# wdykas/LDDL

Measured on AMD Instinct MI355X. Metric: WordPiece+MLM tokens/sec (1/2/4/8 MI355X) and % of HBM roofline, higher is better.
Workload: dtype uint16

## Files before the change

lddl_amd/csrc/tokenize.hip:

```cpp
#include <algorithm>
#include <cstdlib>
#include <cstring>
#include <type_traits>
#include <vector>
#include <cstdio>

#include "common.h"
#include "ctx.h"
#include "device.h"
#include "lddl_amd.h"

namespace lddl {
namespace {

constexpr int kBlock = 128;
constexpr int kWordStride = 420;

__device__ inline uint32_t tab_entry(const Tables& T, uint32_t cp) {
  if (cp > 0x10FFFF) return kDrop << 30;
  return T.pages[(uint32_t)T.l1[cp >> 8] * 256u + (cp & 255u)];
}

__device__ inline uint32_t utf8_next(const uint8_t* b, int64_t end, int64_t& i) {
  const uint32_t c = b[i];
// ... 165 lines not shown
__device__ inline uint64_t lanes_below() { return (1ull << lane_id()) - 1ull; }

__device__ inline int match_special_at(const Tables& T, const uint8_t* b, int64_t i, int64_t end) {
  for (int k = 0; k < kNumSpecial; ++k)
    if (T.special_id[k] >= 0 && match_special(b, i, end, k)) return k;
  return -1;
}

struct B32 {
  uint64_t w0, w1, w2, w3;
};

__device__ inline B32 shr_bytes(const B32& v, int s) {
  const int q = s >> 3, r = (s & 7) * 8;
  uint64_t a0 = q == 0 ? v.w0 : q == 1 ? v.w1 : q == 2 ? v.w2 : v.w3;
  uint64_t a1 = q == 0 ? v.w1 : q == 1 ? v.w2 : q == 2 ? v.w3 : 0ull;
  uint64_t a2 = q == 0 ? v.w2 : q == 1 ? v.w3 : 0ull;
  uint64_t a3 = q == 0 ? v.w3 : 0ull;
  if (r) {
    a0 = (a0 >> r) | (a1 << (64 - r));
    a1 = (a1 >> r) | (a2 << (64 - r));
    a2 = (a2 >> r) | (a3 << (64 - r));
    a3 >>= r;
  }
  return B32{a0, a1, a2, a3};
}

struct Pcs {
  int32_t* b;
  __device__ void put(int n, int32_t v) { b[64 * n] = v; }
  __device__ int32_t get(int q) const { return b[64 * q]; }
};

struct TokStats {
#ifdef LDDL_STAMPS
  uint64_t c[10];
  __device__ void add(int i, uint64_t v) { c[i] += v; }
  __device__ void wave(int i) {
    const uint64_t m = __builtin_amdgcn_ballot_w64(true);
    if ((uint32_t)__lane_id() == (uint32_t)__builtin_ctzll(m)) c[i] += 1;
  }
#else
  __device__ void add(int, uint64_t) {}
  __device__ void wave(int) {}
#endif
};

__device__ inline bool tail_match(const Tables& T, int32_t id, const B32& a, int len) {
  const ulonglong2* p = reinterpret_cast<const ulonglong2*>(T.vlong + 4 * (int64_t)id);
  const ulonglong2 lo = p[0], hi = p[1];
  const uint64_t d = keep_bytes(lo.y ^ a.w1, len - 8) | keep_bytes(hi.x ^ a.w2, len - 16) |
                     keep_bytes(hi.y ^ a.w3, len - 24);
  return d == 0;
}


struct Probe {
  uint64_t k0;
  uint32_t k1, want, slot;
  VEnt e;
};
__device__ inline Probe probe_first(const Tables& T, const B32& a, int len, uint32_t cont) {
  Probe q;
  q.k0 = keep_bytes(a.w0, len);
  q.k1 = (uint32_t)keep_bytes(a.w1, len - 8 < 4 ? len - 8 : 4);
  q.want = kMetaValid | (cont ? kMetaCont : 0u) | (len > 12 ? kMetaLong : 0u) | ((uint32_t)len << 21);
  q.slot = (uint32_t)vhash(q.k0, q.k1, len, cont) & T.vmask;
  q.e = T.vhash[q.slot];
  return q;
// ... 254 lines not shown
  while (j < je) {
    const uint32_t b0 = text[j];
    uint32_t cp, e;
    if (b0 < 0x80) {
      cp = b0;
      e = s_ascii[b0];
      ++j;
    } else {
      cp = utf8_next(text, je, j);
      e = tab_entry(T, cp);
    }
    if ((e >> 30) == kDrop) continue;
    uint8_t ob[12];
    int olen;
    if (e & kIdent) olen = put_utf8(ob, cp);
    else if (e & kMulti) {
      const uint8_t* p = T.pool + (e & 0xFFFFFFu);
      olen = p[0];
      for (int q = 0; q < olen; ++q) ob[q] = p[2 + q];
    } else olen = put_utf8(ob, e & 0x1FFFFFu);
    if (nb + olen > kNorm) return -1;
    for (int q = 0; q < olen; ++q) w[nb + q] = ob[q];
    nb += olen;
  }
  if (nb == 0) return 0;
  uint64_t ends = 1ull << nb;
  for (int e = 1; e < nb; ++e)
    if ((w[e] & 0xC0) != 0x80) ends |= 1ull << e;
  const uint64_t* w8 = reinterpret_cast<const uint64_t*>(w);
  const B32 v{w8[0], w8[1], w8[2], w8[3]};
  return wordpiece32(T, bloom, v, nb, ends, pc);
}

struct UnitWord {
  B32 v;
  int nb;
  uint64_t ends;
  int status;
};

__device__ UnitWord unit_word(const Tables& T, const uint32_t* s_ascii, const uint8_t* __restrict__ text,
                              int64_t n_bytes, int64_t start, int len, bool unit_slow, uint8_t* w) {
  UnitWord u;
  u.status = 0;
  if (!unit_slow && len <= 32 && T.ascii_mode != 0) {
    B32 v = load32(text, n_bytes, start);
    if (T.ascii_mode == 1) v = B32{swar_lower(v.w0), swar_lower(v.w1), swar_lower(v.w2), swar_lower(v.w3)};
    u.v = v;
    u.nb = len;
    u.ends = ~0ull;
    return u;
  }
  int nb = 0;
  int64_t j = start;
  const int64_t je = start + len;
  while (j < je) {
    const uint32_t b0 = text[j];
    uint32_t cp, e;
    if (b0 < 0x80) {
      cp = b0;
      e = s_ascii[b0];
      ++j;
    } else {
      cp = utf8_next(text, je, j);
      e = tab_entry(T, cp);
    }
    if ((e >> 30) == kDrop) continue;
    uint8_t ob[12];
    int olen;
    if (e & kIdent) olen = put_utf8(ob, cp);
    else if (e & kMulti) {
      const uint8_t* p = T.pool + (e & 0xFFFFFFu);
      olen = p[0];
      for (int q = 0; q < olen; ++q) ob[q] = p[2 + q];
    } else olen = put_utf8(ob, e & 0x1FFFFFu);
    if (nb + olen > kNorm) {
      u.status = -1;
      return u;
    }
    for (int q = 0; q < olen; ++q) w[nb + q] = ob[q];
    nb += olen;
  }
  u.nb = nb;
  if (nb == 0) {
    u.status = 1;
    return u;
  }
  uint64_t ends = 1ull << nb;
  for (int e = 1; e < nb; ++e)
    if ((w[e] & 0xC0) != 0x80) ends |= 1ull << e;
  u.ends = ends;
  const uint64_t* w8 = reinterpret_cast<const uint64_t*>(w);
  u.v = B32{w8[0], w8[1], w8[2], w8[3]};
  return u;
}

__global__ void __launch_bounds__(64 * kTW) tokenize_wave_kernel(
    Tables T, const uint8_t* __restrict__ text, int64_t n_bytes, const int64_t* __restrict__ sent_off,
    int64_t n_sent, int32_t max_pieces, int32_t* __restrict__ ids, int32_t* __restrict__ sent_len,
    int32_t* __restrict__ fb_list, uint32_t* __restrict__ fb_n) {
  __shared__ uint32_t s_ascii[128];
  __shared__ WaveLds s_w[kTW];
  for (int c = threadIdx.x; c < 128; c += blockDim.x) s_ascii[c] = tab_entry(T, (uint32_t)c);
  __syncthreads();
  const int lane = lane_id();
  WaveLds& W = s_w[threadIdx.x >> 6];
  const int64_t stride = (int64_t)gridDim.x * kTW;
  for (int64_t s = (int64_t)blockIdx.x * kTW + wave_id(); s < n_sent; s += stride) {
    const int64_t b0 = sent_off[s], b1 = sent_off[s + 1];
    int64_t pos = b0;
    int32_t emitted = 0, flags = 0;
    bool fallback = false;
    while (pos < b1 && emitted < max_pieces) {
      const uint32_t byte = pos + lane < b1 ? text[pos + lane] : 0x20u;
      const WinResult R = classify_window(T, s_ascii, text, pos, b1, byte);
      if (R.fallback) { fallback = true; break; }
      store_units(R, W);
      int npc = 0;
      bool cs_flag = false;
      Pcs pc{W.pcs + lane};
      if (lane < R.n_units) {
        const int us = W.us[lane], ue = W.ue[lane], kind = W.uk[lane];
        const int ulen = ue - us + 1;
        const bool unit_slow = ((R.slow >> us) & (ulen >= 64 ? ~0ull : ((1ull << ulen) - 1))) != 0;
        npc = unit_pieces(T, T.bloom, s_ascii, text, n_bytes, pos + us, ulen, kind, unit_slow, pc,
                          W.nrm + lane * kNorm, cs_flag);
// ... 13 lines not shown
    } else if (lane == 0) {
      sent_len[s] = (emitted < max_pieces ? emitted : max_pieces) | flags;
    }
  }
}

enum : int { kMemoOff = 0, kMemoBuild = 1, kMemoLookup = 2 };
constexpr int kMemoLog2 = 22;
constexpr int kMemoDiv = 32;
struct WordMemo {
  uint4* tab;
  uint32_t mask;
};
constexpr uint32_t kMemoReady = 1u << 31, kMemoClaim = 1u << 30;
__device__ inline B32 memo_key(const B32& v, int nb) {
  return B32{keep_bytes(v.w0, nb), keep_bytes(v.w1, nb - 8), keep_bytes(v.w2, nb - 16),
             keep_bytes(v.w3, nb - 24)};
}
__device__ inline uint32_t memo_slot(const B32& k, int nb) {
  uint64_t h = k.w0 * 0x9E3779B97F4A7C15ull ^ (uint64_t)nb;
  h = (h ^ (h >> 29) ^ k.w1) * 0xBF58476D1CE4E5B9ull;
  h = (h ^ (h >> 32) ^ k.w2) * 0x94D049BB133111EBull;
  h = (h ^ (h >> 29) ^ k.w3) * 0x9E3779B97F4A7C15ull;
  return (uint32_t)(h >> 32);
}

constexpr int kSF = 192;
constexpr int kQ = kSF + 128;
constexpr int kBW = 16;
constexpr int kChunk = 128;
static_assert((kChunk & (kChunk - 1)) == 0, "binary search over the chunk's sentences");
using HIdx = std::conditional_t<(kSF > 256), uint16_t, uint8_t>;
constexpr int32_t kHardBit = INT32_MIN;
constexpr int32_t kQPos = (1 << 28) - 1;
constexpr int32_t kQSlow = INT32_MIN;
constexpr int64_t kMaxSpan = 1 << 28;
constexpr int32_t kRFb = 1 << 29;
constexpr int32_t kRCnt = kRFb - 1;
static_assert(kLenHasClsSep == (1 << 30), "r_cnt flag layout");
enum : uint32_t { kFRun = 0, kFSep = 1, kFIso = 2, kFSlow = 4 };

struct alignas(16) StreamLds {
  int32_t q_s[kQ];
  int32_t q_e[kQ];
  uint8_t q_slot[kQ];
  int32_t q_res[kSF];
  uint8_t q_npc[kSF];
  HIdx h_idx[kSF];
  int32_t s_off[kChunk + 1];
  int32_t r_cnt[kChunk];
  alignas(16) int32_t pcs[kPcs * 64];
};
static_assert(kPcs * 64 * 4 >= 64 * kNorm, "normalised-word rows must fit the piece columns");

#ifdef LDDL_STAMPS
__device__ unsigned long long* g_tok_tl;
__device__ unsigned long long* g_tok_reg;
constexpr int kTokRegions = 6;
#define TOK_STAMP(r)                                                     \
  do {                                                                   \
    const unsigned long long _now = __builtin_amdgcn_s_memtime();       \
    reg_acc[r] += _now - reg_last;                                       \
    reg_last = _now;                                                     \
  } while (0)
#else
#define TOK_STAMP(r) \
  do {               \
  } while (0)
#endif

template <int kMemo>
__global__ void __launch_bounds__(64 * kBW, 1) tokenize_batch_kernel(
    Tables T_arg, const uint8_t* __restrict__ text, int64_t n_bytes, const int64_t* __restrict__ sent_off,
    int64_t n_sent, int32_t max_pieces, int32_t* __restrict__ ids, int32_t* __restrict__ sent_len_arg,
    int32_t* __restrict__ fb_list_arg, uint32_t* __restrict__ fb_n_arg, int32_t* __restrict__ chunk_ctr_arg,
    WordMemo M) {
  __shared__ uint32_t s_ascii[128];
  __shared__ uint8_t s_cls[256];
  __shared__ uint32_t s_bloom[kBloomWords];
  __shared__ StreamLds s_w[kBW];
  __shared__ Tables s_T;
  __shared__ int32_t* s_cold[4];
  if (threadIdx.x == 0) {
    s_T = T_arg;
    s_cold[0] = sent_len_arg;
    s_cold[1] = fb_list_arg;
    s_cold[2] = reinterpret_cast<int32_t*>(fb_n_arg);
    s_cold[3] = chunk_ctr_arg;
  }
  __syncthreads();
  const Tables& T = s_T;
  int32_t* const volatile* cold = s_cold;
#ifdef LDDL_STAMPS
  const unsigned long long rt0 = __builtin_amdgcn_s_memrealtime();
  unsigned long long reg_acc[kTokRegions] = {0, 0, 0, 0, 0, 0};
  unsigned long long reg_last = __builtin_amdgcn_s_memtime();
  TokStats tstat;
  for (int q = 0; q < 10; ++q) tstat.c[q] = 0;
  TokStats* tsp = &tstat;
#else
  TokStats* tsp = nullptr;
#endif
  for (int c = threadIdx.x; c < 128; c += blockDim.x) s_ascii[c] = tab_entry(T, (uint32_t)c);
  for (int c = threadIdx.x; c < 256; c += blockDim.x) {
    uint32_t v = kFSlow;
    if (c < 128 && c != '[') {
      const uint32_t cl = tab_entry(T, (uint32_t)c) >> 30;
      v = cl == kSpace ? kFSep : cl == kIso ? kFIso : cl == kWord ? kFRun : kFSlow;
    }
    s_cls[c] = (uint8_t)v;
  }
  for (int c = threadIdx.x; c < kBloomWords; c += blockDim.x) s_bloom[c] = T.bloom[c];
  __syncthreads();
  const int lane = lane_id();
  StreamLds& W = s_w[threadIdx.x >> 6];
  int32_t* const trashp = &W.pcs[lane_id()];
  const int32_t n_sent32 = (int32_t)n_sent;
  int32_t c0;
  {
    const int64_t w = (int64_t)blockIdx.x * kBW + (threadIdx.x >> 6);
    c0 = __builtin_amdgcn_readfirstlane(w * kChunk < n_sent32 ? (int32_t)(w * kChunk) : n_sent32);
  }
  const uint64_t upto = (2ull << lane) - 1;

  while (c0 < n_sent32) {
    const int32_t n = n_sent32 - c0 < kChunk ? n_sent32 - c0 : kChunk;
    const int64_t A = sent_off[c0];
    const int64_t span64 = sent_off[c0 + n] - A;
    if (span64 >= kMaxSpan) {
      for (int j = lane; j < n; j += 64)
        cold[1][atomicAdd(reinterpret_cast<uint32_t*>(cold[2]), 1u)] = c0 + j;
// ... 94 lines not shown
              lenr[r] = len;
              if (kind >= 2) {
                resr[r] = T.special_id[kind - 2];
              } else if (qs >= 0 && T.ascii_mode != 0 && len <= T.max_piece_bytes && len <= 32) {
                elig[r] = true;
                vv[r] = load32(text, n_bytes, A + st);
              } else {
                hardr[r] = true;
              }
            }
          }
#pragma unroll
          for (int r = 0; r < kR; ++r)
            if (elig[r]) {
              if (T.ascii_mode == 1)
                vv[r] = B32{swar_lower(vv[r].w0), swar_lower(vv[r].w1), swar_lower(vv[r].w2), swar_lower(vv[r].w3)};
              pr[r] = probe_first(T, vv[r], lenr[r], 0);
            }
#pragma unroll
          for (int r = 0; r < kR; ++r) {
            if (elig[r]) {
              resr[r] = probe_finish(T, vv[r], lenr[r], pr[r]);
              hardr[r] = resr[r] < 0;
            }
            const int u = 64 * r + lane;
            if (u < m && !hardr[r]) {
              W.q_res[u] = resr[r];
              W.q_npc[u] = 1;
            }
            const uint64_t H = ballot(hardr[r]);
            if (hardr[r]) {
              const int k = nh + (int)popc_below(H);
              W.h_idx[k] = (HIdx)u;
              if (elig[r] && k < 64) {
                uint4* row = reinterpret_cast<uint4*>(reinterpret_cast<uint8_t*>(W.pcs) + 32 * k);
                row[0] = make_uint4((uint32_t)vv[r].w0, (uint32_t)(vv[r].w0 >> 32), (uint32_t)vv[r].w1,
                                    (uint32_t)(vv[r].w1 >> 32));
                row[1] = make_uint4((uint32_t)vv[r].w2, (uint32_t)(vv[r].w2 >> 32), (uint32_t)vv[r].w3,
                                    (uint32_t)(vv[r].w3 >> 32));
              }
            }
            nh += __popcll(H);
          }
        }
        wave_sync();
        TOK_STAMP(1);
        int placed = 0;
        if (tsp) {
          tsp->wave(8);
          tsp->add(9, lane == 0 ? m : 0);
        }
        for (int h0 = 0; h0 < nh; h0 += 64) {
          const int hn = nh - h0 < 64 ? nh - h0 : 64;
          if (tsp) {
            tsp->wave(0);
            tsp->add(1, lane < hn);
          }
          int u = -1, st = 0;
          UnitWord uw;
          uw.status = 1;
          bool known_miss = false;
          if (lane < hn) {
            u = W.h_idx[h0 + lane];
            const int32_t qs = W.q_s[u];
            st = qs & kQPos;
            const int len = W.q_e[u] - st + 1;
            const bool slow = qs < 0;
            known_miss = !slow && T.ascii_mode != 0 && len <= T.max_piece_bytes && len <= 32;
            if (h0 == 0 && known_miss) {
              const uint4* row = reinterpret_cast<const uint4*>(reinterpret_cast<const uint8_t*>(W.pcs) + 32 * lane);
              const uint4 r0 = row[0], r1 = row[1];
              uw.v = B32{r0.x | (uint64_t)r0.y << 32, r0.z | (uint64_t)r0.w << 32,
                         r1.x | (uint64_t)r1.y << 32, r1.z | (uint64_t)r1.w << 32};
              uw.nb = len;
              uw.ends = ~0ull;
              uw.status = 0;
            } else {
              uw = unit_word(T, s_ascii, text, n_bytes, A + st, len, slow,
                             reinterpret_cast<uint8_t*>(W.pcs) + 32 * lane);
            }
          }
          wave_sync();
          int npc = 0;
          if (lane < hn) {
            Pcs pc{W.pcs + lane};
            if (uw.status == 0) {
              if constexpr (kMemo == kMemoOff) {
                npc = wordpiece32(T, s_bloom, uw.v, uw.nb, uw.ends, pc, known_miss, tsp);
              } else {
                const B32 key = memo_key(uw.v, uw.nb);
                uint4* e = M.tab + 4 * (size_t)(memo_slot(key, uw.nb) & M.mask);
                bool hit = false;
                if constexpr (kMemo == kMemoLookup) {
                  const uint4 k0 = e[0], k1 = e[1], pz = e[2];
                  const uint32_t meta = e[3].x;
                  hit = (meta & kMemoReady) && (int)(meta & 0xFFu) == uw.nb &&
                        ((k0.x | (uint64_t)k0.y << 32) ^ key.w0 | (k0.z | (uint64_t)k0.w << 32) ^ key.w1 |
                         (k1.x | (uint64_t)k1.y << 32) ^ key.w2 | (k1.z | (uint64_t)k1.w << 32) ^ key.w3) == 0;
                  if (hit) {
                    npc = (int)((meta >> 8) & 0xFu);
                    const uint32_t pw[4] = {pz.x, pz.y, pz.z, pz.w};
#pragma unroll
                    for (int q = 0; q < kPcs; ++q)
                      if (q < npc) pc.put(q, (int32_t)((pw[q >> 1] >> (16 * (q & 1))) & 0xFFFFu));
                  }
                }
                if (!hit) npc = wordpiece32(T, s_bloom, uw.v, uw.nb, uw.ends, pc, known_miss, tsp);
                if constexpr (kMemo == kMemoBuild) {
                  if (npc >= 1 && atomicCAS(&e[3].x, 0u, kMemoClaim) == 0u) {
                    uint32_t pw[4] = {0u, 0u, 0u, 0u};
#pragma unroll
                    for (int q = 0; q < kPcs; ++q)
                      if (q < npc) pw[q >> 1] |= ((uint32_t)pc.get(q) & 0xFFFFu) << (16 * (q & 1));
                    e[0] = make_uint4((uint32_t)key.w0, (uint32_t)(key.w0 >> 32), (uint32_t)key.w1,
                                      (uint32_t)(key.w1 >> 32));
                    e[1] = make_uint4((uint32_t)key.w2, (uint32_t)(key.w2 >> 32), (uint32_t)key.w3,
                                      (uint32_t)(key.w3 >> 32));
                    e[2] = make_uint4(pw[0], pw[1], pw[2], pw[3]);
                    e[3].x = kMemoReady | (uint32_t)uw.nb | (uint32_t)npc << 8;
                  }
                }
              }
            } else if (uw.status < 0) {
              npc = -1;
            }
            if (npc < 0) {
              atomicOr(&W.r_cnt[sent_of(st)], kRFb);
              npc = 0;
            }
            W.q_res[u] = kHardBit | lane;
            W.q_npc[u] = (uint8_t)npc;
          }
          wave_sync();
          const int lim = h0 + 64 < nh ? (int)W.h_idx[h0 + 64] : m;
          TOK_STAMP(2);
          place(placed, lim);
          placed = lim;
          TOK_STAMP(3);
        }
        place(placed, m);
        TOK_STAMP(3);
        drop(m);
        TOK_STAMP(4);
      };

      uint64_t UNITp = 0, CONTp = 0;
      uint64_t cin = 0;
      uint32_t cpack = 0, plcp = 0;
      int32_t jn = 1;
      uint32_t nextS = (uint32_t)__builtin_amdgcn_readfirstlane(W.s_off[1]);
      const uint32_t last = span ? span - 1 : 0;
      uint32_t cur = 0x20u, pf1 = 0x20u, pf2 = 0x20u;
      if (span) {
        cur = ctext[(uint32_t)lane < last ? (uint32_t)lane : last];
        pf1 = ctext[64u + lane < last ? 64u + lane : last];
        pf2 = ctext[128u + lane < last ? 128u + lane : last];
      }
      uint32_t x0 = 0;
      for (; x0 < span; x0 += 64) {
        const uint32_t byte = cur;
        const uint32_t v = s_cls[byte];
        cur = pf1;
        pf1 = pf2;
        {
          const uint32_t xq = x0 + 192u + lane;
          pf2 = ctext[xq < last ? xq : last];
        }
        const uint32_t x = x0 + lane;
// ... 97 lines not shown
        if (ne >= kSF) {
          wave_sync();
          flush(kSF);
        }
      }
      {
        const uint64_t UEp = UNITp & ~(CONTp >> 1);
        const uint32_t r = popc_below(UEp) + (uint32_t)ne;
        int32_t* dst = ((UEp >> lane) & 1ull) ? &W.q_e[r] : trashp;
        *dst = (int32_t)(x0 - 64u + lane);
        ne += (int)__popcll(UEp);
      }
      wave_sync();
      TOK_STAMP(0);
      while (ne > 0) flush(ne < kSF ? ne : kSF);
      for (int j = lane; j < n; j += 64) {
        const int32_t rc = W.r_cnt[j];
        if (rc & kRFb) {
          cold[1][atomicAdd(reinterpret_cast<uint32_t*>(cold[2]), 1u)] = c0 + j;
        } else {
          const int32_t cnt = rc & kRCnt;
          cold[0][c0 + j] = (cnt < max_pieces ? cnt : max_pieces) | (rc & kLenHasClsSep);
        }
      }
      wave_sync();
    }
    TOK_STAMP(5);
    int32_t nc = 0;
    if (lane == 0) nc = atomicAdd(cold[3], kChunk);
    nc = __builtin_amdgcn_readfirstlane(nc);
    c0 = nc < n_sent32 ? nc : n_sent32;
  }
#ifdef LDDL_STAMPS
  if (lane == 0 && g_tok_tl) {
    const int64_t wv = (int64_t)blockIdx.x * kBW + (threadIdx.x >> 6);
    g_tok_tl[2 * wv] = rt0;
    g_tok_tl[2 * wv + 1] = __builtin_amdgcn_s_memrealtime();
  }
  if (lane == 0 && g_tok_reg)
    for (int r = 0; r < kTokRegions; ++r) atomicAdd(g_tok_reg + r, reg_acc[r]);
  if (g_tok_reg)
    for (int q = 0; q < 10; ++q) {
      const uint64_t v = wave_sum(tstat.c[q]);
      if (lane == 0) atomicAdd(g_tok_reg + kTokRegions + q, (unsigned long long)v);
    }
#endif
}

}
}

using namespace lddl;

constexpr int kFbHead = 1;

struct TokCall {
  lddl_ctx* c;
  hipStream_t st;
  const uint8_t* d_text;
  int64_t n_bytes;
  const int64_t* d_sent_off;
  int64_t n_sent;
  int32_t max_pieces;
  int32_t* d_ids;
  int32_t* d_sent_len;
  int32_t* fb = nullptr;
  int32_t* chunk_ctr = nullptr;
  int64_t n_cu = 256;
  int64_t grid = 0;
};

static int launch_lane(const TokCall& T, int64_t s0, int64_t n, int64_t grid_cap, bool whole) {
  const int64_t grid = std::min<int64_t>((n + kBlock - 1) / kBlock, grid_cap);
  hipLaunchKernelGGL(tokenize_lane_kernel, dim3((unsigned)grid), dim3(kBlock), 0, T.st, T.c->tab,
                     T.d_text, T.d_sent_off + s0, n, T.max_pieces, T.d_ids, T.d_sent_len + s0,
                     whole ? nullptr : T.fb + kFbHead,
                     whole ? nullptr : reinterpret_cast<const uint32_t*>(T.fb));
  LDDL_HIP(hipGetLastError());
  return 0;
}

static int tokenize_wave(const TokCall& T) {
  int per_cu = 0;
  LDDL_HIP(hipOccupancyMaxActiveBlocksPerMultiprocessor(&per_cu, tokenize_wave_kernel, 64 * kTW, 0));
  const int64_t want = (T.n_sent + kTW - 1) / kTW;
  const int64_t grid = std::min<int64_t>(want, T.n_cu * std::max(per_cu, 1));
  hipLaunchKernelGGL(tokenize_wave_kernel, dim3((unsigned)grid), dim3(64 * kTW), 0, T.st, T.c->tab,
                     T.d_text, T.n_bytes, T.d_sent_off, T.n_sent, T.max_pieces, T.d_ids, T.d_sent_len,
                     T.fb + kFbHead, reinterpret_cast<uint32_t*>(T.fb));
  return launch_lane(T, 0, T.n_sent, T.n_cu * 2, false);
}

static int batch_pass(TokCall& T, int64_t grid_max, int64_t s0, int64_t n, int memo, WordMemo M) {
  const int64_t want = (n + 16 * kBW - 1) / (16 * kBW);
  int64_t grid = std::max<int64_t>(1, std::min<int64_t>(want, grid_max));
  if (const char* g = getenv("LDDL_TOKENIZE_GRID")) grid = std::max<int64_t>(1, std::min<int64_t>(grid, atoll(g)));
  T.grid = grid;
  const int64_t first = std::min<int64_t>(grid * kBW * kChunk, (int64_t)INT32_MAX);
  LDDL_HIP(hipMemsetAsync(T.fb, 0, sizeof(int32_t) * kFbHead, T.st));
  LDDL_HIP(hipMemsetD32Async(reinterpret_cast<hipDeviceptr_t>(T.chunk_ctr), (int)first, 1, T.st));
  const void* kfn = memo == kMemoBuild ? (const void*)tokenize_batch_kernel<kMemoBuild>
                  : memo == kMemoLookup ? (const void*)tokenize_batch_kernel<kMemoLookup>
                                        : (const void*)tokenize_batch_kernel<kMemoOff>;
  const int64_t* so = T.d_sent_off + s0;
  int32_t* sl = T.d_sent_len + s0;
  int32_t* fl = T.fb + kFbHead;
  uint32_t* fn = reinterpret_cast<uint32_t*>(T.fb);
  void* args[] = {&T.c->tab, (void*)&T.d_text, &T.n_bytes, (void*)&so, &n, &T.max_pieces, &T.d_ids, &sl,
                  &fl, &fn, &T.chunk_ctr, &M};
  LDDL_HIP(hipLaunchKernel(kfn, dim3((unsigned)grid), dim3(64 * kBW), args, 0, T.st));
  return launch_lane(T, s0, n, T.n_cu * 2, false);
}

#ifdef LDDL_STAMPS
static int stamps_begin(ArenaScope& diag, const TokCall& T, int64_t grid_max, unsigned long long** tl,
                        unsigned long long** rg) {
  int rc;
  if ((rc = diag.take(tl, 2 * grid_max * kBW)) || (rc = diag.take(rg, kTokRegions + 10))) return rc;
  LDDL_HIP(hipMemsetAsync(*tl, 0, 16 * grid_max * kBW, T.st));
  LDDL_HIP(hipMemcpyToSymbolAsync(HIP_SYMBOL(g_tok_tl), tl, sizeof(*tl), 0, hipMemcpyHostToDevice, T.st));
  LDDL_HIP(hipMemsetAsync(*rg, 0, 8 * (kTokRegions + 10), T.st));
  LDDL_HIP(hipMemcpyToSymbolAsync(HIP_SYMBOL(g_tok_reg), rg, sizeof(*rg), 0, hipMemcpyHostToDevice, T.st));
  return 0;
}

static int report_tok_stamps(const TokCall& T, const unsigned long long* tl, const unsigned long long* rg) {
  const int64_t nw = T.grid * kBW;
  std::vector<unsigned long long> t(2 * nw);
  LDDL_HIP(hipMemcpyAsync(t.data(), tl, 16 * nw, hipMemcpyDeviceToHost, T.st));
  LDDL_HIP(hipStreamSynchronize(T.st));
  unsigned long long t0 = ~0ull, t1 = 0;
  std::vector<double> e(nw);
  for (int64_t q = 0; q < nw; ++q) {
    t0 = std::min(t0, t[2 * q]);
    t1 = std::max(t1, t[2 * q + 1]);
  }
  for (int64_t q = 0; q < nw; ++q) e[q] = (t[2 * q + 1] - t0) / 1e5;
  std::sort(e.begin(), e.end());
  const double span = (t1 - t0) / 1e5;
  fprintf(stderr, "[tok timeline] span %.2f ms, wave end ms: min %.2f p10 %.2f p50 %.2f p90 %.2f max %.2f\n",
          span, e[0], e[nw / 10], e[nw / 2], e[nw * 9 / 10], e[nw - 1]);
  const int nb = 40;
  fprintf(stderr, "[tok timeline] waves alive per %.2f ms bin:", span / nb);
  for (int b = 0; b < nb; ++b) {
    const double te = span * (b + 0.5) / nb;
    int64_t alive = 0;
    for (int64_t q = 0; q < nw; ++q) alive += e[q] > te;
    fprintf(stderr, " %lld", (long long)alive);
  }
  fprintf(stderr, "\n");
  unsigned long long r[kTokRegions + 10];
  LDDL_HIP(hipMemcpy(r, rg, sizeof r, hipMemcpyDeviceToHost));
  const unsigned long long* k = r + kTokRegions;
  fprintf(stderr,
          "[tok phaseB] flushes %llu units %llu | passes %llu lanes/pass %.1f | piece-steps: wave %llu "
          "lane %llu (lane util %.2f) | bloom iters: wave %llu lane-useful %llu (util %.2f, per wave "
          "step %.1f) | probe trips: wave %llu lane %llu (util %.2f)\n",
          k[8], k[9], k[0], (double)k[1] / (k[0] ? k[0] : 1), k[2], k[3],
          (double)k[3] / (64.0 * (k[2] ? k[2] : 1)), k[4], k[5], (double)k[5] / (64.0 * (k[4] ? k[4] : 1)),
          (double)k[4] / (k[2] ? k[2] : 1), k[6], k[7], (double)k[7] / (64.0 * (k[6] ? k[6] : 1)));
  unsigned long long tot = 0;
  for (int q = 0; q < kTokRegions; ++q) tot += r[q];
  static const char* names[kTokRegions] = {"banks", "phaseA", "phaseB", "place", "qshift", "chunk"};
  fprintf(stderr, "[tok regions] wave-cycle shares:");
  for (int q = 0; q < kTokRegions; ++q) fprintf(stderr, " %s %.1f%%", names[q], 100.0 * r[q] / (tot ? tot : 1));
  fprintf(stderr, "\n");
  return 0;
}
#endif

extern "C" int lddl_tokenize(lddl_ctx* c, void* stream, const uint8_t* d_text, int64_t n_bytes,
                             const int64_t* d_sent_off, int64_t n_sent, int32_t max_pieces,
                             int32_t* d_ids, int32_t* d_sent_len) {
  if (!c) LDDL_FAIL(-1, "null ctx");
  if (n_sent < 0 || n_bytes < 0 || max_pieces <= 0 || max_pieces > (1 << 24))
    LDDL_FAIL(-1, "bad sizes (max_pieces must be in 1 .. 2^24)");
  if (n_sent >= (int64_t)INT32_MAX - (1 << 22)) LDDL_FAIL(-1, "too many sentences in one call (%lld)", (long long)n_sent);
  if (n_sent == 0) return 0;
  hipStream_t st = as_stream(stream);
  TokCall T{c, st, d_text, n_bytes, d_sent_off, n_sent, max_pieces, d_ids, d_sent_len};
  const char* path = getenv("LDDL_TOKENIZE_PATH");
  if (path && !strcmp(path, "lane")) return launch_lane(T, 0, n_sent, 65536, true);
  if (path && strcmp(path, "wave") && strcmp(path, "fused") && strcmp(path, "plain"))
    LDDL_FAIL(-1, "LDDL_TOKENIZE_PATH must be lane, wave, fused or plain (got %s)", path);
  ArenaTmp fbb(&c->arena, st);
  LDDL_HIP(fbb.take(sizeof(int32_t) * (size_t)(n_sent + kFbHead + 1)));
  T.fb = fbb.as<int32_t>();
  T.chunk_ctr = T.fb + kFbHead + n_sent;
  LDDL_HIP(hipMemsetAsync(T.fb, 0, sizeof(int32_t) * kFbHead, st));
  int n_cu = 256;
  (void)hipDeviceGetAttribute(&n_cu, hipDeviceAttributeMultiprocessorCount, c->device);
  T.n_cu = n_cu;
  if (path && !strcmp(path, "wave")) return tokenize_wave(T);
  int per_cu = 0;
  LDDL_HIP(hipOccupancyMaxActiveBlocksPerMultiprocessor(&per_cu, tokenize_batch_kernel<kMemoOff>, 64 * kBW, 0));
  const int64_t grid_max = T.n_cu * std::max(per_cu, 1);
  int rc;
#ifdef LDDL_STAMPS
  ArenaScope diag(&c->arena, st);
  unsigned long long *tl, *rg;
  if ((rc = stamps_begin(diag, T, grid_max, &tl, &rg))) return rc;
#endif
  constexpr int64_t kMemoMinSample = 1 << 14;
  int64_t n_sample = std::max<int64_t>(n_sent / kMemoDiv, kMemoMinSample);
  bool memo = c->vocab_size <= 65536 && n_sent >= 4 * kMemoMinSample;
  if (const char* e = getenv("LDDL_TOKENIZE_MEMO_SAMPLE")) {
    n_sample = atoll(e);
    memo = c->vocab_size <= 65536 && n_sample > 0 && n_sample < n_sent;
  }
  if (path && !strcmp(path, "plain")) memo = false;
  if (!memo) {
    if ((rc = batch_pass(T, grid_max, 0, n_sent, kMemoOff, WordMemo{nullptr, 0}))) return rc;
  } else {
    ArenaTmp mb(&c->arena, st);
    const size_t entries = (size_t)1 << kMemoLog2;
    LDDL_HIP(mb.take(64 * entries));
    LDDL_HIP(hipMemsetAsync(mb.as<void>(), 0, 64 * entries, st));
// ... 11 lines not shown
```

Baseline: 71.85 billion.

## Normalise short non-ASCII words in registers and precompute row-cache flags

Adds a register-based normaliser for words of at most 32 bytes containing up to four non-ASCII codepoints. It decodes UTF-8 from one 32-byte load and batches the table lookups, replacing the byte-by-byte global-memory loop in the slow path. The piece-end bitmask is now computed with SWAR bit tricks instead of a per-byte loop, and a per-unit flag in LDS records known-miss and cached-row status so later passes do not recompute them. The memo lookup is restructured and more diagnostic counters are added; the register path adds code size and register pressure to a kernel that runs one workgroup per CU.

```diff
diff --git a/lddl_amd/csrc/tokenize.hip b/lddl_amd/csrc/tokenize.hip
--- a/lddl_amd/csrc/tokenize.hip
+++ b/lddl_amd/csrc/tokenize.hip
@@ -221,9 +221,10 @@
   __device__ int32_t get(int q) const { return b[64 * q]; }
 };
 
+[[maybe_unused]] constexpr int kTokCounters = 12;
 struct TokStats {
 #ifdef LDDL_STAMPS
-  uint64_t c[10];
+  uint64_t c[kTokCounters];
   __device__ void add(int i, uint64_t v) { c[i] += v; }
   __device__ void wave(int i) {
     const uint64_t m = __builtin_amdgcn_ballot_w64(true);
@@ -544,6 +545,107 @@
   return wordpiece32(T, bloom, v, nb, ends, pc);
 }
 
+constexpr int kSlowCps = 4;
+constexpr uint64_t k80 = 0x8080808080808080ull;
+
+__device__ inline uint32_t byte_at(const B32& v, int j) {
+  const uint64_t w = j < 8 ? v.w0 : j < 16 ? v.w1 : j < 24 ? v.w2 : v.w3;
+  return (uint32_t)(w >> (8 * (j & 7))) & 0xFFu;
+}
+
+__device__ inline uint32_t top_bits(uint64_t t) {
+  return (uint32_t)(((t >> 7) * 0x0102040810204080ull) >> 56);
+}
+__device__ inline uint32_t top_bits32(const B32& t) {
+  return top_bits(t.w0) | top_bits(t.w1) << 8 | top_bits(t.w2) << 16 | top_bits(t.w3) << 24;
+}
+
+__device__ inline uint32_t utf8_next_regs(const B32& v, int end, int& i) {
+  const uint32_t c = byte_at(v, i);
+  if (c < 0x80) { ++i; return c; }
+  const int len = c >= 0xF0 ? 4 : c >= 0xE0 ? 3 : c >= 0xC0 ? 2 : 1;
+  if (len == 1 || i + len > end) { ++i; return 0xFFFD; }
+  uint32_t cp = c & (0x7Fu >> len);
+  for (int k = 1; k < len; ++k) {
+    const uint32_t d = byte_at(v, i + k);
+    if ((d & 0xC0) != 0x80) { ++i; return 0xFFFD; }
+    cp = (cp << 6) | (d & 0x3F);
+  }
+  i += len;
+  return cp;
+}
+
+__device__ __forceinline__ int norm_regs(const Tables& T, const uint32_t* s_ascii, const uint8_t* __restrict__ text,
+                         int64_t n_bytes, int64_t start, int len, uint8_t* w) {
+  const B32 raw = load32(text, n_bytes, start);
+  const uint32_t in_unit = len >= 32 ? ~0u : (1u << len) - 1u;
+  const uint32_t hi = top_bits32(B32{raw.w0 & k80, raw.w1 & k80, raw.w2 & k80, raw.w3 & k80}) & in_unit;
+  uint32_t cp[kSlowCps], ent[kSlowCps], advs = 0, rest = hi;
+#pragma unroll
+  for (int k = 0; k < kSlowCps; ++k) {
+    cp[k] = 0;
+    if (rest) {
+      const int j = __builtin_ctz(rest);
+      int i = j;
+      cp[k] = utf8_next_regs(raw, len, i);
+      advs |= (uint32_t)(i - j) << (3 * k);
+      rest = i >= 32 ? 0u : rest & (~0u << i);
+    }
+  }
+  if (rest) return -2;
+#ifdef LDDL_SLOW_BATCH
+  {
+    uint32_t page[kSlowCps];
+#pragma unroll
+    for (int k = 0; k < kSlowCps; ++k) page[k] = T.l1[cp[k] > 0x10FFFFu ? 0u : cp[k] >> 8];
+    static_assert(kSlowCps == 4, "the dependency below names four");
+    asm volatile("" : "+v"(page[0]), "+v"(page[1]), "+v"(page[2]), "+v"(page[3]));
+#pragma unroll
+    for (int k = 0; k < kSlowCps; ++k) ent[k] = T.pages[page[k] * 256u + (cp[k] & 255u)];
+#pragma unroll
+    for (int k = 0; k < kSlowCps; ++k)
+      if (cp[k] > 0x10FFFFu) ent[k] = kDrop << 30;
+  }
+#else
+#pragma unroll
+  for (int k = 0; k < kSlowCps; ++k) {
+    ent[k] = 0;
+    if (advs >> (3 * k)) ent[k] = tab_entry(T, cp[k]);
+  }
+#endif
+  int nb = 0;
+  for (int j = 0; j < len;) {
+    uint32_t c, e;
+    if (!((hi >> j) & 1u)) {
+      c = byte_at(raw, j);
+      e = s_ascii[c];
+      ++j;
+    } else {
+      c = cp[0];
+      e = ent[0];
+      j += (int)(advs & 7u);
+      advs >>= 3;
+#pragma unroll
+      for (int k = 0; k + 1 < kSlowCps; ++k) cp[k] = cp[k + 1], ent[k] = ent[k + 1];
+    }
+    if ((e >> 30) == kDrop) continue;
+    if (!(e & kIdent) && (e & kMulti)) {
+      const uint8_t* p = T.pool + (e & 0xFFFFFFu);
+      const int olen = p[0];
+      if (nb + olen > kNorm) return -1;
+      for (int q = 0; q < olen; ++q) w[nb + q] = p[2 + q];
+      nb += olen;
+    } else {
+      const uint32_t o = (e & kIdent) ? c : e & 0x1FFFFFu;
+      const int olen = o < 0x80 ? 1 : o < 0x800 ? 2 : o < 0x10000 ? 3 : 4;
+      if (nb + olen > kNorm) return -1;
+      put_utf8(w + nb, o);
+      nb += olen;
+    }
+  }
+  return nb;
+}
+
 struct UnitWord {
   B32 v;
   int nb;
@@ -551,8 +653,9 @@
   int status;
 };
 
-__device__ UnitWord unit_word(const Tables& T, const uint32_t* s_ascii, const uint8_t* __restrict__ text,
-                              int64_t n_bytes, int64_t start, int len, bool unit_slow, uint8_t* w) {
+__device__ __forceinline__ UnitWord unit_word(const Tables& T, const uint32_t* s_ascii, const uint8_t* __restrict__ text,
+                              int64_t n_bytes, int64_t start, int len, bool unit_slow, uint8_t* w,
+                              bool regs) {
   UnitWord u;
   u.status = 0;
   if (!unit_slow && len <= 32 && T.ascii_mode != 0) {
@@ -563,47 +666,50 @@
     u.ends = ~0ull;
     return u;
   }
-  int nb = 0;
-  int64_t j = start;
-  const int64_t je = start + len;
-  while (j < je) {
-    const uint32_t b0 = text[j];
-    uint32_t cp, e;
-    if (b0 < 0x80) {
-      cp = b0;
-      e = s_ascii[b0];
-      ++j;
-    } else {
-      cp = utf8_next(text, je, j);
-      e = tab_entry(T, cp);
-    }
-    if ((e >> 30) == kDrop) continue;
-    uint8_t ob[12];
-    int olen;
-    if (e & kIdent) olen = put_utf8(ob, cp);
-    else if (e & kMulti) {
-      const uint8_t* p = T.pool + (e & 0xFFFFFFu);
-      olen = p[0];
-      for (int q = 0; q < olen; ++q) ob[q] = p[2 + q];
-    } else olen = put_utf8(ob, e & 0x1FFFFFu);
-    if (nb + olen > kNorm) {
-      u.status = -1;
-      return u;
-    }
-    for (int q = 0; q < olen; ++q) w[nb + q] = ob[q];
-    nb += olen;
+  int nb = -2;
+  if (regs && len <= 32 && T.ascii_mode != 0) nb = norm_regs(T, s_ascii, text, n_bytes, start, len, w);
+  if (nb == -2) {
+    nb = 0;
+    int64_t j = start;
+    const int64_t je = start + len;
+    while (j < je) {
+      const uint32_t b0 = text[j];
+      uint32_t cp, e;
+      if (b0 < 0x80) {
+        cp = b0;
+        e = s_ascii[b0];
+        ++j;
+      } else {
+        cp = utf8_next(text, je, j);
+        e = tab_entry(T, cp);
+      }
+      if ((e >> 30) == kDrop) continue;
+      uint8_t ob[12];
+      int olen;
+      if (e & kIdent) olen = put_utf8(ob, cp);
+      else if (e & kMulti) {
+        const uint8_t* p = T.pool + (e & 0xFFFFFFu);
+        olen = p[0];
+        for (int q = 0; q < olen; ++q) ob[q] = p[2 + q];
+      } else olen = put_utf8(ob, e & 0x1FFFFFu);
+      if (nb + olen > kNorm) {
+        nb = -1;
+        break;
+      }
+      for (int q = 0; q < olen; ++q) w[nb + q] = ob[q];
+      nb += olen;
+    }
   }
   u.nb = nb;
-  if (nb == 0) {
-    u.status = 1;
+  if (nb <= 0) {
+    u.status = nb < 0 ? -1 : 1;
     return u;
   }
-  uint64_t ends = 1ull << nb;
-  for (int e = 1; e < nb; ++e)
-    if ((w[e] & 0xC0) != 0x80) ends |= 1ull << e;
-  u.ends = ends;
   const uint64_t* w8 = reinterpret_cast<const uint64_t*>(w);
   u.v = B32{w8[0], w8[1], w8[2], w8[3]};
+  const uint32_t cont = top_bits32(B32{u.v.w0 & ~(u.v.w0 << 1) & k80, u.v.w1 & ~(u.v.w1 << 1) & k80,
+                                       u.v.w2 & ~(u.v.w2 << 1) & k80, u.v.w3 & ~(u.v.w3 << 1) & k80});
+  u.ends = ((uint64_t)(~cont & ~1u) & ((1ull << nb) - 1ull)) | 1ull << nb;
   return u;
 }
 
@@ -683,6 +789,8 @@
 static_assert((kChunk & (kChunk - 1)) == 0, "binary search over the chunk's sentences");
 using HIdx = std::conditional_t<(kSF > 256), uint16_t, uint8_t>;
 constexpr int32_t kHardBit = INT32_MIN;
+constexpr uint32_t kRowMiss = 1u;
+constexpr uint32_t kRowValid = 2u;
 constexpr int32_t kQPos = (1 << 28) - 1;
 constexpr int32_t kQSlow = INT32_MIN;
 constexpr int64_t kMaxSpan = 1 << 28;
@@ -707,17 +815,27 @@
 #ifdef LDDL_STAMPS
 __device__ unsigned long long* g_tok_tl;
 __device__ unsigned long long* g_tok_reg;
-constexpr int kTokRegions = 6;
+constexpr int kTokRegions = 10;
+constexpr int kTokDiag = kTokRegions + kTokCounters;
+constexpr int kTokSlices = 2;
+constexpr int kTokTlWgs = 1024;
 #define TOK_STAMP(r)                                                     \
   do {                                                                   \
     const unsigned long long _now = __builtin_amdgcn_s_memtime();       \
     reg_acc[r] += _now - reg_last;                                       \
     reg_last = _now;                                                     \
   } while (0)
+#define TOK_STAMP_SPLIT(r) \
+  }                        \
+  }                        \
+  TOK_STAMP(r);            \
+  if (lane < hn) {         \
+    if (uw.status == 0) {
 #else
 #define TOK_STAMP(r) \
   do {               \
   } while (0)
+#define TOK_STAMP_SPLIT(r)
 #endif
 
 template <int kMemo>
@@ -725,15 +843,17 @@
     Tables T_arg, const uint8_t* __restrict__ text, int64_t n_bytes, const int64_t* __restrict__ sent_off,
     int64_t n_sent, int32_t max_pieces, int32_t* __restrict__ ids, int32_t* __restrict__ sent_len_arg,
     int32_t* __restrict__ fb_list_arg, uint32_t* __restrict__ fb_n_arg, int32_t* __restrict__ chunk_ctr_arg,
-    WordMemo M) {
+    WordMemo M, int32_t slow_loop_arg) {
   __shared__ uint32_t s_ascii[128];
   __shared__ uint8_t s_cls[256];
   __shared__ uint32_t s_bloom[kBloomWords];
   __shared__ StreamLds s_w[kBW];
   __shared__ Tables s_T;
   __shared__ int32_t* s_cold[4];
+  __shared__ int32_t s_slow_loop;
   if (threadIdx.x == 0) {
     s_T = T_arg;
+    s_slow_loop = slow_loop_arg;
     s_cold[0] = sent_len_arg;
     s_cold[1] = fb_list_arg;
     s_cold[2] = reinterpret_cast<int32_t*>(fb_n_arg);
@@ -744,10 +864,10 @@
   int32_t* const volatile* cold = s_cold;
 #ifdef LDDL_STAMPS
   const unsigned long long rt0 = __builtin_amdgcn_s_memrealtime();
-  unsigned long long reg_acc[kTokRegions] = {0, 0, 0, 0, 0, 0};
+  unsigned long long reg_acc[kTokRegions] = {0, 0, 0, 0, 0, 0, 0, 0, 0, 0};
   unsigned long long reg_last = __builtin_amdgcn_s_memtime();
   TokStats tstat;
-  for (int q = 0; q < 10; ++q) tstat.c[q] = 0;
+  for (int q = 0; q < kTokCounters; ++q) tstat.c[q] = 0;
   TokStats* tsp = &tstat;
 #else
   TokStats* tsp = nullptr;
@@ -908,6 +1028,7 @@
             if (hardr[r]) {
               const int k = nh + (int)popc_below(H);
               W.h_idx[k] = (HIdx)u;
+              W.q_npc[u] = (uint8_t)(!elig[r] ? 0u : k < 64 ? kRowMiss | kRowValid : kRowMiss);
               if (elig[r] && k < 64) {
                 uint4* row = reinterpret_cast<uint4*>(reinterpret_cast<uint8_t*>(W.pcs) + 32 * k);
                 row[0] = make_uint4((uint32_t)vv[r].w0, (uint32_t)(vv[r].w0 >> 32), (uint32_t)vv[r].w1,
@@ -942,8 +1063,13 @@
             st = qs & kQPos;
             const int len = W.q_e[u] - st + 1;
             const bool slow = qs < 0;
-            known_miss = !slow && T.ascii_mode != 0 && len <= T.max_piece_bytes && len <= 32;
-            if (h0 == 0 && known_miss) {
+            const uint32_t note = W.q_npc[u];
+            known_miss = (note & kRowMiss) != 0;
+            if (tsp) {
+              tsp->add(10, slow);
+              if (ballot(slow)) tsp->wave(11);
+            }
+            if (note & kRowValid) {
               const uint4* row = reinterpret_cast<const uint4*>(reinterpret_cast<const uint8_t*>(W.pcs) + 32 * lane);
               const uint4 r0 = row[0], r1 = row[1];
               uw.v = B32{r0.x | (uint64_t)r0.y << 32, r0.z | (uint64_t)r0.w << 32,
@@ -953,48 +1079,52 @@
               uw.status = 0;
             } else {
               uw = unit_word(T, s_ascii, text, n_bytes, A + st, len, slow,
-                             reinterpret_cast<uint8_t*>(W.pcs) + 32 * lane);
+                             reinterpret_cast<uint8_t*>(W.pcs) + 32 * lane, !s_slow_loop);
             }
           }
           wave_sync();
+          TOK_STAMP(6);
           int npc = 0;
+          bool hit = false;
+          Pcs pc{W.pcs + lane};
           if (lane < hn) {
-            Pcs pc{W.pcs + lane};
             if (uw.status == 0) {
-              if constexpr (kMemo == kMemoOff) {
-                npc = wordpiece32(T, s_bloom, uw.v, uw.nb, uw.ends, pc, known_miss, tsp);
-              } else {
-                const B32 key = memo_key(uw.v, uw.nb);
+              if constexpr (kMemo != kMemoOff) {
+                uw.v = memo_key(uw.v, uw.nb);
+              }
+              if constexpr (kMemo == kMemoLookup) {
+                const B32& key = uw.v;
+                const uint4* e = M.tab + 4 * (size_t)(memo_slot(key, uw.nb) & M.mask);
+                const uint4 k0 = e[0], k1 = e[1], pz = e[2];
+                const uint32_t meta = e[3].x;
+                hit = (meta & kMemoReady) && (int)(meta & 0xFFu) == uw.nb &&
+                      (((k0.x | (uint64_t)k0.y << 32) ^ key.w0) | ((k0.z | (uint64_t)k0.w << 32) ^ key.w1) |
+                       ((k1.x | (uint64_t)k1.y << 32) ^ key.w2) | ((k1.z | (uint64_t)k1.w << 32) ^ key.w3)) == 0;
+                if (hit) {
+                  npc = (int)((meta >> 8) & 0xFu);
+                  const uint32_t pw[4] = {pz.x, pz.y, pz.z, pz.w};
+#pragma unroll
+                  for (int q = 0; q < kPcs; ++q)
+                    if (q < npc) pc.put(q, (int32_t)((pw[q >> 1] >> (16 * (q & 1))) & 0xFFFFu));
+                }
+              }
+              TOK_STAMP_SPLIT(7);
+              if (!hit) npc = wordpiece32(T, s_bloom, uw.v, uw.nb, uw.ends, pc, known_miss, tsp);
+              TOK_STAMP_SPLIT(8);
+              if constexpr (kMemo == kMemoBuild) {
+                const B32& key = uw.v;
                 uint4* e = M.tab + 4 * (size_t)(memo_slot(key, uw.nb) & M.mask);
-                bool hit = false;
-                if constexpr (kMemo == kMemoLookup) {
-                  const uint4 k0 = e[0], k1 = e[1], pz = e[2];
-                  const uint32_t meta = e[3].x;
-                  hit = (meta & kMemoReady) && (int)(meta & 0xFFu) == uw.nb &&
-                        ((k0.x | (uint64_t)k0.y << 32) ^ key.w0 | (k0.z | (uint64_t)k0.w << 32) ^ key.w1 |
-                         (k1.x | (uint64_t)k1.y << 32) ^ key.w2 | (k1.z | (uint64_t)k1.w << 32) ^ key.w3) == 0;
-                  if (hit) {
-                    npc = (int)((meta >> 8) & 0xFu);
-                    const uint32_t pw[4] = {pz.x, pz.y, pz.z, pz.w};
+                if (npc >= 1 && atomicCAS(&e[3].x, 0u, kMemoClaim) == 0u) {
+                  uint32_t pw[4] = {0u, 0u, 0u, 0u};
 #pragma unroll
-                    for (int q = 0; q < kPcs; ++q)
-                      if (q < npc) pc.put(q, (int32_t)((pw[q >> 1] >> (16 * (q & 1))) & 0xFFFFu));
-                  }
-                }
-                if (!hit) npc = wordpiece32(T, s_bloom, uw.v, uw.nb, uw.ends, pc, known_miss, tsp);
-                if constexpr (kMemo == kMemoBuild) {
-                  if (npc >= 1 && atomicCAS(&e[3].x, 0u, kMemoClaim) == 0u) {
-                    uint32_t pw[4] = {0u, 0u, 0u, 0u};
-#pragma unroll
-                    for (int q = 0; q < kPcs; ++q)
-                      if (q < npc) pw[q >> 1] |= ((uint32_t)pc.get(q) & 0xFFFFu) << (16 * (q & 1));
-                    e[0] = make_uint4((uint32_t)key.w0, (uint32_t)(key.w0 >> 32), (uint32_t)key.w1,
-                                      (uint32_t)(key.w1 >> 32));
-                    e[1] = make_uint4((uint32_t)key.w2, (uint32_t)(key.w2 >> 32), (uint32_t)key.w3,
-                                      (uint32_t)(key.w3 >> 32));
-                    e[2] = make_uint4(pw[0], pw[1], pw[2], pw[3]);
-                    e[3].x = kMemoReady | (uint32_t)uw.nb | (uint32_t)npc << 8;
-                  }
+                  for (int q = 0; q < kPcs; ++q)
+                    if (q < npc) pw[q >> 1] |= ((uint32_t)pc.get(q) & 0xFFFFu) << (16 * (q & 1));
+                  e[0] = make_uint4((uint32_t)key.w0, (uint32_t)(key.w0 >> 32), (uint32_t)key.w1,
+                                    (uint32_t)(key.w1 >> 32));
+                  e[1] = make_uint4((uint32_t)key.w2, (uint32_t)(key.w2 >> 32), (uint32_t)key.w3,
+                                    (uint32_t)(key.w3 >> 32));
+                  e[2] = make_uint4(pw[0], pw[1], pw[2], pw[3]);
+                  e[3].x = kMemoReady | (uint32_t)uw.nb | (uint32_t)npc << 8;
                 }
               }
             } else if (uw.status < 0) {
@@ -1009,7 +1139,7 @@
           }
           wave_sync();
           const int lim = h0 + 64 < nh ? (int)W.h_idx[h0 + 64] : m;
-          TOK_STAMP(2);
+          TOK_STAMP(9);
           place(placed, lim);
           placed = lim;
           TOK_STAMP(3);
@@ -1173,17 +1303,19 @@
     c0 = nc < n_sent32 ? nc : n_sent32;
   }
 #ifdef LDDL_STAMPS
+  constexpr int slice = kMemo == kMemoLookup ? 1 : 0;
   if (lane == 0 && g_tok_tl) {
-    const int64_t wv = (int64_t)blockIdx.x * kBW + (threadIdx.x >> 6);
+    const int64_t wv = ((int64_t)slice * kTokTlWgs + blockIdx.x) * kBW + (threadIdx.x >> 6);
     g_tok_tl[2 * wv] = rt0;
     g_tok_tl[2 * wv + 1] = __builtin_amdgcn_s_memrealtime();
   }
-  if (lane == 0 && g_tok_reg)
-    for (int r = 0; r < kTokRegions; ++r) atomicAdd(g_tok_reg + r, reg_acc[r]);
-  if (g_tok_reg)
-    for (int q = 0; q < 10; ++q) {
+  unsigned long long* const reg = g_tok_reg ? g_tok_reg + slice * kTokDiag : nullptr;
+  if (lane == 0 && reg)
+    for (int r = 0; r < kTokRegions; ++r) atomicAdd(reg + r, reg_acc[r]);
+  if (reg)
+    for (int q = 0; q < kTokCounters; ++q) {
       const uint64_t v = wave_sum(tstat.c[q]);
-      if (lane == 0) atomicAdd(g_tok_reg + kTokRegions + q, (unsigned long long)v);
+      if (lane == 0) atomicAdd(reg + kTokRegions + q, (unsigned long long)v);
     }
 #endif
 }
@@ -1209,6 +1341,8 @@
   int32_t* chunk_ctr = nullptr;
   int64_t n_cu = 256;
   int64_t grid = 0;
+  int64_t grid_of[2] = {0, 0};
+  int32_t slow_loop = 0;
 };
 
 static int launch_lane(const TokCall& T, int64_t s0, int64_t n, int64_t grid_cap, bool whole) {
@@ -1237,6 +1371,7 @@
   int64_t grid = std::max<int64_t>(1, std::min<int64_t>(want, grid_max));
   if (const char* g = getenv("LDDL_TOKENIZE_GRID")) grid = std::max<int64_t>(1, std::min<int64_t>(grid, atoll(g)));
   T.grid = grid;
+  T.grid_of[memo == kMemoLookup ? 1 : 0] = grid;
   const int64_t first = std::min<int64_t>(grid * kBW * kChunk, (int64_t)INT32_MAX);
   LDDL_HIP(hipMemsetAsync(T.fb, 0, sizeof(int32_t) * kFbHead, T.st));
   LDDL_HIP(hipMemsetD32Async(reinterpret_cast<hipDeviceptr_t>(T.chunk_ctr), (int)first, 1, T.st));
@@ -1248,7 +1383,7 @@
   int32_t* fl = T.fb + kFbHead;
   uint32_t* fn = reinterpret_cast<uint32_t*>(T.fb);
   void* args[] = {&T.c->tab, (void*)&T.d_text, &T.n_bytes, (void*)&so, &n, &T.max_pieces, &T.d_ids, &sl,
-                  &fl, &fn, &T.chunk_ctr, &M};
+                  &fl, &fn, &T.chunk_ctr, &M, &T.slow_loop};
   LDDL_HIP(hipLaunchKernel(kfn, dim3((unsigned)grid), dim3(64 * kBW), args, 0, T.st));
   return launch_lane(T, s0, n, T.n_cu * 2, false);
 }
@@ -1256,17 +1391,20 @@
 #ifdef LDDL_STAMPS
 static int stamps_begin(ArenaScope& diag, const TokCall& T, int64_t grid_max, unsigned long long** tl,
                         unsigned long long** rg) {
+  if (grid_max > kTokTlWgs) LDDL_FAIL(-1, "diagnostic build: %lld workgroups exceed kTokTlWgs", (long long)grid_max);
+  const size_t n_tl = (size_t)2 * kTokSlices * kTokTlWgs * kBW, n_rg = (size_t)kTokSlices * kTokDiag;
   int rc;
-  if ((rc = diag.take(tl, 2 * grid_max * kBW)) || (rc = diag.take(rg, kTokRegions + 10))) return rc;
-  LDDL_HIP(hipMemsetAsync(*tl, 0, 16 * grid_max * kBW, T.st));
+  if ((rc = diag.take(tl, n_tl)) || (rc = diag.take(rg, n_rg))) return rc;
+  LDDL_HIP(hipMemsetAsync(*tl, 0, 8 * n_tl, T.st));
   LDDL_HIP(hipMemcpyToSymbolAsync(HIP_SYMBOL(g_tok_tl), tl, sizeof(*tl), 0, hipMemcpyHostToDevice, T.st));
-  LDDL_HIP(hipMemsetAsync(*rg, 0, 8 * (kTokRegions + 10), T.st));
+  LDDL_HIP(hipMemsetAsync(*rg, 0, 8 * n_rg, T.st));
   LDDL_HIP(hipMemcpyToSymbolAsync(HIP_SYMBOL(g_tok_reg), rg, sizeof(*rg), 0, hipMemcpyHostToDevice, T.st));
   return 0;
 }
 
-static int report_tok_stamps(const TokCall& T, const unsigned long long* tl, const unsigned long long* rg) {
-  const int64_t nw = T.grid * kBW;
+static int report_tok_slice(const TokCall& T, const char* label, int64_t grid, const unsigned long long* tl,
+                            const unsigned long long* rg) {
+  const int64_t nw = grid * kBW;
   std::vector<unsigned long long> t(2 * nw);
   LDDL_HIP(hipMemcpyAsync(t.data(), tl, 16 * nw, hipMemcpyDeviceToHost, T.st));
   LDDL_HIP(hipStreamSynchronize(T.st));
@@ -1279,10 +1417,10 @@
   for (int64_t q = 0; q < nw; ++q) e[q] = (t[2 * q + 1] - t0) / 1e5;
   std::sort(e.begin(), e.end());
   const double span = (t1 - t0) / 1e5;
-  fprintf(stderr, "[tok timeline] span %.2f ms, wave end ms: min %.2f p10 %.2f p50 %.2f p90 %.2f max %.2f\n",
-          span, e[0], e[nw / 10], e[nw / 2], e[nw * 9 / 10], e[nw - 1]);
+  fprintf(stderr, "[tok %s timeline] span %.2f ms, wave end ms: min %.2f p10 %.2f p50 %.2f p90 %.2f max %.2f\n",
+          label, span, e[0], e[nw / 10], e[nw / 2], e[nw * 9 / 10], e[nw - 1]);
   const int nb = 40;
-  fprintf(stderr, "[tok timeline] waves alive per %.2f ms bin:", span / nb);
+  fprintf(stderr, "[tok %s timeline] waves alive per %.2f ms bin:", label, span / nb);
   for (int b = 0; b < nb; ++b) {
     const double te = span * (b + 0.5) / nb;
     int64_t alive = 0;
@@ -1290,22 +1428,41 @@
     fprintf(stderr, " %lld", (long long)alive);
   }
   fprintf(stderr, "\n");
-  unsigned long long r[kTokRegions + 10];
+  unsigned long long r[kTokDiag];
   LDDL_HIP(hipMemcpy(r, rg, sizeof r, hipMemcpyDeviceToHost));
   const unsigned long long* k = r + kTokRegions;
   fprintf(stderr,
-          "[tok phaseB] flushes %llu units %llu | passes %llu lanes/pass %.1f | piece-steps: wave %llu "
+          "[tok %s phaseB] flushes %llu units %llu | passes %llu lanes/pass %.1f | piece-steps: wave %llu "
           "lane %llu (lane util %.2f) | bloom iters: wave %llu lane-useful %llu (util %.2f, per wave "
-          "step %.1f) | probe trips: wave %llu lane %llu (util %.2f)\n",
-          k[8], k[9], k[0], (double)k[1] / (k[0] ? k[0] : 1), k[2], k[3],
+          "step %.1f) | probe trips: wave %llu lane %llu (util %.2f) | slow lanes %llu (%.2f per pass), "
+          "passes with one %llu (%.1f%%)\n",
+          label, k[8], k[9], k[0], (double)k[1] / (k[0] ? k[0] : 1), k[2], k[3],
           (double)k[3] / (64.0 * (k[2] ? k[2] : 1)), k[4], k[5], (double)k[5] / (64.0 * (k[4] ? k[4] : 1)),
-          (double)k[4] / (k[2] ? k[2] : 1), k[6], k[7], (double)k[7] / (64.0 * (k[6] ? k[6] : 1)));
+          (double)k[4] / (k[2] ? k[2] : 1), k[6], k[7], (double)k[7] / (64.0 * (k[6] ? k[6] : 1)), k[10],
+          (double)k[10] / (k[0] ? k[0] : 1), k[11], 100.0 * k[11] / (k[0] ? k[0] : 1));
+  r[2] = r[6] + r[7] + r[8] + r[9];
   unsigned long long tot = 0;
-  for (int q = 0; q < kTokRegions; ++q) tot += r[q];
-  static const char* names[kTokRegions] = {"banks", "phaseA", "phaseB", "place", "qshift", "chunk"};
-  fprintf(stderr, "[tok regions] wave-cycle shares:");
-  for (int q = 0; q < kTokRegions; ++q) fprintf(stderr, " %s %.1f%%", names[q], 100.0 * r[q] / (tot ? tot : 1));
-  fprintf(stderr, "\n");
+  for (int q = 0; q < 6; ++q) tot += r[q];
+  static const char* names[kTokRegions] = {"banks", "phaseA", "phaseB", "place", "qshift", "chunk",
+                                           "B0 fetch+normalise", "B1 memo", "B2 greedy", "B3 rest"};
+  fprintf(stderr, "[tok %s regions] wave-cycle shares:", label);
+  for (int q = 0; q < 6; ++q) fprintf(stderr, " %s %.1f%%", names[q], 100.0 * r[q] / (tot ? tot : 1));
+  fprintf(stderr, "\n[tok %s phaseB split] share of phase B (of the kernel):", label);
+  for (int q = 6; q < kTokRegions; ++q)
+    fprintf(stderr, " %s %.1f%% (%.1f%%)", names[q], 100.0 * r[q] / (r[2] ? r[2] : 1), 100.0 * r[q] / (tot ? tot : 1));
+  fprintf(stderr, " | phase-B wave cycles per pass %.0f\n", (double)r[2] / (k[0] ? k[0] : 1));
+  return 0;
+}
+
+static int report_tok_stamps(const TokCall& T, const unsigned long long* tl, const unsigned long long* rg) {
+  static const char* labels[2][kTokSlices] = {{"single", ""}, {"build", "lookup"}};
+  const bool two = T.grid_of[1] > 0;
+  for (int s = 0; s < kTokSlices; ++s) {
+    if (!T.grid_of[s]) continue;
+    int rc = report_tok_slice(T, labels[two][s], T.grid_of[s], tl + (size_t)2 * s * kTokTlWgs * kBW,
+                              rg + (size_t)s * kTokDiag);
+    if (rc) return rc;
+  }
   return 0;
 }
 #endif
@@ -1324,6 +1481,11 @@
   if (path && !strcmp(path, "lane")) return launch_lane(T, 0, n_sent, 65536, true);
   if (path && strcmp(path, "wave") && strcmp(path, "fused") && strcmp(path, "plain"))
     LDDL_FAIL(-1, "LDDL_TOKENIZE_PATH must be lane, wave, fused or plain (got %s)", path);
+  if (const char* sl = getenv("LDDL_TOKENIZE_SLOW")) {
+    if (strcmp(sl, "regs") && strcmp(sl, "loop"))
+      LDDL_FAIL(-1, "LDDL_TOKENIZE_SLOW must be regs or loop (got %s)", sl);
+    T.slow_loop = !strcmp(sl, "loop");
+  }
   ArenaTmp fbb(&c->arena, st);
   LDDL_HIP(fbb.take(sizeof(int32_t) * (size_t)(n_sent + kFbHead + 1)));
   T.fb = fbb.as<int32_t>();
```

After: 72.90 billion (median of 6 runs). 1.01x the previous value.
